# jjjkkyz/NU-NeRF

Hardware: AMD Instinct MI355X
Metric: train rays/sec (higher is better)
Workload: dtype f32

## Files before the change

### nu_nerf_amd/build.py

```python
import hashlib
import os
import subprocess
import sys

HERE = os.path.dirname(os.path.abspath(__file__))
CSRC = os.path.join(HERE, "csrc")
LIB = os.path.join(HERE, "libnunerf.so")
STAMP = os.path.join(HERE, ".libnunerf.stamp")
HIPCC = os.environ.get("HIPCC", "/opt/rocm/bin/hipcc")
FLAGS = ["--offload-arch=gfx950", "-O3", "-std=c++17", "-fPIC",
         "-fno-gpu-rdc", "-Wno-unused-result", "-I" + CSRC, "-I" + os.path.join(HERE, "..", "include")]
if os.environ.get("NU_BUILD_NO_PK_F32", "0") == "1":
    FLAGS += ["-Xclang", "-target-feature", "-Xclang", "-packed-fp32-ops"]


def _sources():
    return sorted(os.path.join(CSRC, f) for f in os.listdir(CSRC) if f.endswith(".hip"))


def _digest():
    h = hashlib.sha256()
    for f in sorted(os.listdir(CSRC)):
        if f.endswith((".hip", ".h")):
            with open(os.path.join(CSRC, f), "rb") as fh:
                h.update(f.encode())
                h.update(fh.read())
    inc = os.path.join(HERE, "..", "include", "nu_nerf.h")
    if os.path.exists(inc):
        with open(inc, "rb") as fh:
            h.update(fh.read())
    h.update(" ".join(FLAGS).encode())
    return h.hexdigest()


def build(force=False, verbose=True):
    dig = _digest()
    if not force and os.path.exists(LIB) and os.path.exists(STAMP):
        with open(STAMP) as fh:
            if fh.read().strip() == dig:
                return LIB
    objs = []
    procs = []
    objdir = os.path.join(HERE, "build")
    os.makedirs(objdir, exist_ok=True)
    for src in _sources():
        obj = os.path.join(objdir, os.path.basename(src)[:-4] + ".o")
        objs.append(obj)
        cmd = [HIPCC] + FLAGS + ["-c", src, "-o", obj]
        if verbose:
            print(" ".join(cmd), flush=True)
        procs.append((src, subprocess.Popen(cmd)))
    for src, p in procs:
        if p.wait() != 0:
            raise RuntimeError(f"hipcc failed on {src}")
    cmd = [HIPCC, "--offload-arch=gfx950", "-shared", "-fPIC", "-o", LIB] + objs
    if verbose:
        print(" ".join(cmd), flush=True)
    subprocess.check_call(cmd)
    with open(STAMP, "w") as fh:
        fh.write(dig)
    return LIB


if __name__ == "__main__":
    build(force="--force" in sys.argv)
    print(LIB)
```

### nu_nerf_amd/csrc/gemm_tn.hip

```cpp
#include "gemm_epi.h"

__device__ unsigned long long nu_dbg_clk[2];

#define NU_TN_BATCH_MAX 16
struct NuGemmTNBatch {
    NuGemmTN p[NU_TN_BATCH_MAX];
    int blk0[NU_TN_BATCH_MAX + 1];
    int n, pad_;
};
static __device__ __forceinline__ int tn_batch_decode(const NuGemmTNBatch& b, int tile_edge, int& bx, int& split) {
    int pi = 0;
    for (int i = 1; i < b.n; ++i) pi = ((int)blockIdx.x >= b.blk0[i]) ? i : pi;
    const int tiles = ((b.p[pi].N1 + tile_edge - 1) / tile_edge) * ((b.p[pi].N2 + tile_edge - 1) / tile_edge);
    const int local = (int)blockIdx.x - b.blk0[pi];
    split = local / tiles;
    bx = local - split * tiles;
    return pi;
}

template <bool BIG, int PREC>
static __device__ __forceinline__ void tn_body(const NuGemmTN& g, const int bx, const int split, const int grp) {
    constexpr bool BF16 = PREC == 1;
    constexpr bool SPLIT = PREC == 2;
    constexpr int kPlane = 128 * NT_LDSH;
    __shared__ __attribute__((aligned(16))) float smem[SPLIT ? 1 : 2][SPLIT ? 3 * kPlane : 128 * NT_LDS];
    __bf16* const hA = reinterpret_cast<__bf16*>(&smem[0][0]);
    __bf16* const hB = hA + (SPLIT ? 3 : 1) * kPlane;

    const int tid = threadIdx.x;
    const int lane = tid & 63;
    const int wid = tid >> 6;
    const int wr = wid >> 1, wc = wid & 1;
    const int t2 = (g.N2 + 127) / 128;
    const int n1t = bx / t2, n2t = bx - n1t * t2;
    const int n1_0 = n1t * 128, n2_0 = n2t * 128;
    const int N1p = ((g.N1 + 127) / 128) * 128, N2p = t2 * 128;

    int rows_per = (g.P + g.S - 1) / g.S;
    rows_per = ((rows_per + TBK - 1) / TBK) * TBK;
    const int p_begin = split * rows_per;
    int p_end = p_begin + rows_per;
    p_end = p_end < g.P ? p_end : g.P;
    const int ntile = p_end > p_begin ? (p_end - p_begin + TBK - 1) / TBK : 0;
    const int npair = g.A1 ? 2 : 1;
    const int total = ntile * npair;

    const int c = tid & 127;
    const int kg = tid >> 7;
    const bool do_bias = (g.bias_slab != nullptr) && (n2t == 0);

    f32x16 acc[2][2];
#pragma unroll
    for (int i = 0; i < 2; ++i)
#pragma unroll
        for (int j = 0; j < 2; ++j)
#pragma unroll
            for (int r = 0; r < 16; ++r) acc[i][j][r] = 0.0f;

    f32x4 ra4[4], rb4[4];
    int nvalid = 16;
    bool pend_pair0 = true;
    float bs = 0.f;
    auto load_tile = [&](int t) {
        const int pair = t >= ntile ? 1 : 0;
        const int kt = t - pair * ntile;
        const bool a16 = BF16 && (g.bf16 & (pair ? NU_TN_A1_16 : NU_TN_A0_16)) != 0;
        const bool b16 = BF16 && (g.bf16 & (pair ? NU_TN_B1_16 : NU_TN_B0_16)) != 0;
        const unsigned eA = a16 ? 2u : 4u, eB = b16 ? 2u : 4u;
        const char* __restrict__ A = (const char*)(pair ? g.A1 : g.A0) + (long long)grp * (pair ? g.sA1 : g.sA0) * eA;
        const char* __restrict__ B = (const char*)(pair ? g.B1 : g.B0) + (long long)grp * (pair ? g.sB1 : g.sB0) * eB;
        const int lda = pair ? g.lda1 : g.lda0;
        const int ldb = pair ? g.ldb1 : g.ldb0;
        int ca = n1_0 + c, cb = n2_0 + c;
        ca = ca < lda ? ca : lda - 1;
        cb = cb < ldb ? cb : ldb - 1;
        const int pbase = p_begin + kt * TBK + kg * 16;
        nvalid = p_end - pbase;
        pend_pair0 = pair == 0;
#pragma unroll
        for (int i = 0; i < 4; ++i)
#pragma unroll
            for (int e = 0; e < 4; ++e) {
                int pr = pbase + 4 * i + e;
                pr = pr < p_end ? pr : p_end - 1;
                const char* pa;
                const char* pb;
                if (BIG) {
                    pa = A + ((long long)pr * lda + ca) * eA;
                    pb = B + ((long long)pr * ldb + cb) * eB;
                } else {
                    pa = A + ((unsigned)pr * (unsigned)lda + (unsigned)ca) * eA;
                    pb = B + ((unsigned)pr * (unsigned)ldb + (unsigned)cb) * eB;
                }
                ra4[i][e] = a16 ? __uint_as_float((unsigned)*reinterpret_cast<const unsigned short*>(pa) << 16) : *reinterpret_cast<const float*>(pa);
                rb4[i][e] = b16 ? __uint_as_float((unsigned)*reinterpret_cast<const unsigned short*>(pb) << 16) : *reinterpret_cast<const float*>(pb);
            }
    };
    auto store_tile = [&]() {
#pragma unroll
        for (int i = 0; i < 4; ++i)
#pragma unroll
            for (int e = 0; e < 4; ++e) {
                const bool ok = 4 * i + e < nvalid;
                ra4[i][e] = ok ? ra4[i][e] : 0.f;
                rb4[i][e] = ok ? rb4[i][e] : 0.f;
            }
        if (do_bias && pend_pair0) {
#pragma unroll
            for (int i = 0; i < 4; ++i) bs += (ra4[i][0] + ra4[i][1]) + (ra4[i][2] + ra4[i][3]);
        }
#pragma unroll
        for (int i = 0; i < 4; ++i) {
            if (SPLIT) {
                bf16x4 p1, p2, p3;
                nu_split3(ra4[i], p1, p2, p3);
                __bf16* q = &hA[c * NT_LDSH + kg * 16 + 4 * i];
                *reinterpret_cast<bf16x4*>(q) = p1;
                *reinterpret_cast<bf16x4*>(q + kPlane) = p2;
                *reinterpret_cast<bf16x4*>(q + 2 * kPlane) = p3;
                nu_split3(rb4[i], p1, p2, p3);
                q = &hB[c * NT_LDSH + kg * 16 + 4 * i];
                *reinterpret_cast<bf16x4*>(q) = p1;
                *reinterpret_cast<bf16x4*>(q + kPlane) = p2;
                *reinterpret_cast<bf16x4*>(q + 2 * kPlane) = p3;
            } else if (BF16) {
                *reinterpret_cast<bf16x4*>(&hA[c * NT_LDSH + kg * 16 + 4 * i]) = nu_to_bf16x4(ra4[i]);
                *reinterpret_cast<bf16x4*>(&hB[c * NT_LDSH + kg * 16 + 4 * i]) = nu_to_bf16x4(rb4[i]);
            } else {
                float* s0 = &smem[0][0];
                *reinterpret_cast<f32x4*>(&s0[c * NT_LDS + kg * 16 + 4 * i]) = ra4[i];
                *reinterpret_cast<f32x4*>(&s0[128 * NT_LDS + c * NT_LDS + kg * 16 + 4 * i]) = rb4[i];
            }
        }
    };

    if (total > 0) {
        load_tile(0);
        store_tile();
    }
    __syncthreads();

    const int li = lane & 31, lh = lane >> 5;
    const int a_off = (wr * 64 + li) * NT_LDS + 4 * lh;
    const int b_off = (wc * 64 + li) * NT_LDS + 4 * lh;
    const int ah_off = (wr * 64 + li) * NT_LDSH + 8 * lh;
    const int bh_off = (wc * 64 + li) * NT_LDSH + 8 * lh;
    const int wr_u = __builtin_amdgcn_readfirstlane(wr), wc_u = __builtin_amdgcn_readfirstlane(wc);
    const bool vr0 = n1_0 + wr_u * 64 < g.N1, vr1 = n1_0 + wr_u * 64 + 32 < g.N1;
    const bool vc0 = n2_0 + wc_u * 64 < g.N2, vc1 = n2_0 + wc_u * 64 + 32 < g.N2;
    const bool v00 = vr0 && vc0, v01 = vr0 && vc1, v10 = vr1 && vc0, v11 = vr1 && vc1;
    for (int t = 0; t < total; ++t) {
        if (t + 1 < total) load_tile(t + 1);
        if (SPLIT) {
#pragma unroll
            for (int ks = 0; ks < 2; ++ks) {
// ... 501 lines not shown
            const bool ok = 4 * i + e < nvalid;
            ra4[i][e] = ok ? ra4[i][e] : 0.f;
            rb4[i][e] = ok ? rb4[i][e] : 0.f;
        }
        if (do_bias && pend_pair0) bs += (ra4[i][0] + ra4[i][1]) + (ra4[i][2] + ra4[i][3]);
        *reinterpret_cast<f32x4*>(&smem[st][0][c * NT_LDS + kg * 16 + 4 * i]) = ra4[i];
        *reinterpret_cast<f32x4*>(&smem[st][1][c * NT_LDS + kg * 16 + 4 * i]) = rb4[i];
    };
    auto load_tile = [&](int t) {
        load_begin(t);
#pragma unroll
        for (int i = 0; i < 4; ++i) load_piece(i, 0, 4);
        nvalid = nvalid_ld; pend_pair0 = pair0_ld;
    };
    auto store_tile = [&](int st) {
#pragma unroll
        for (int i = 0; i < 4; ++i) store_piece(st, i);
    };

    if (total > 0) {
        load_tile(0);
        store_tile(0);
        if (total > 1) load_tile(1);
    }
    __syncthreads();

    const int li = lane & 31, lh = lane >> 5;
    const int a_off = (wr * 64 + li) * NT_LDS + 4 * lh;
    const int b_off = (wc * 128 + li) * NT_LDS + 4 * lh;
    struct FragT { f32x4 a[2]; f32x4 b[4]; };
    FragT F0, F1;
    const int kg_u = __builtin_amdgcn_readfirstlane(kg);
    const char* rpA = nullptr;
    const char* rpB = nullptr;
    int prA = 0, prB = 0;
    auto ld_rows_begin = [&]() {
        int pr = ld_pbase_u + kg_u * 16;
        pr = pr < p_end ? pr : p_end - 1;
        prA = prB = pr;
        rpA = ldA + (long long)pr * ld_lda * 4;
        rpB = ldB + (long long)pr * ld_ldb * 4;
    };
    auto ld_one = [&](bool isA, int i, int e) {
        if (isA) {
            ra4[i][e] = *reinterpret_cast<const float*>(rpA + (unsigned)ld_ca * 4u);
            const bool more = prA + 1 < p_end;
            rpA += more ? (long long)ld_lda * 4 : 0;
            prA += more ? 1 : 0;
        } else {
            rb4[i][e] = *reinterpret_cast<const float*>(rpB + (unsigned)ld_cb * 4u);
            const bool more = prB + 1 < p_end;
            rpB += more ? (long long)ld_ldb * 4 : 0;
            prB += more ? 1 : 0;
        }
    };
    auto st_zero = [&](bool isA, int i) {
#pragma unroll
        for (int e = 0; e < 4; ++e) {
            if (isA) ra4[i][e] = (4 * i + e < nvalid) ? ra4[i][e] : 0.f;
            else rb4[i][e] = (4 * i + e < nvalid) ? rb4[i][e] : 0.f;
        }
    };
    bool bias_on = false;
    auto st_write = [&](bool isA, int st, int i) {
        if (isA) {
            const float rs = (ra4[i][0] + ra4[i][1]) + (ra4[i][2] + ra4[i][3]);
            bs += bias_on ? rs : 0.f;
            *reinterpret_cast<f32x4*>(&smem[st][0][c * NT_LDS + kg * 16 + 4 * i]) = ra4[i];
        } else {
            *reinterpret_cast<f32x4*>(&smem[st][1][c * NT_LDS + kg * 16 + 4 * i]) = rb4[i];
        }
    };
    int cur = 0;
    if (total > 0) {
#pragma unroll
        for (int i = 0; i < 2; ++i) F0.a[i] = *reinterpret_cast<const f32x4*>(&smem[0][0][a_off + 32 * i * NT_LDS]);
#pragma unroll
        for (int j = 0; j < 4; ++j) F0.b[j] = *reinterpret_cast<const f32x4*>(&smem[0][1][b_off + 32 * j * NT_LDS]);
    }
#define TN_PIN __builtin_amdgcn_sched_barrier(0);
#define TN_M(F, e, i, j) acc[i][j] = __builtin_amdgcn_mfma_f32_32x32x2f32(F.a[i][e], F.b[j][e], acc[i][j], 0, 0, 0); TN_PIN
#define TN_SLOT(F, e, ...) TN_SLOT_(F, e, __VA_ARGS__)
#define TN_SLOT_(F, e, X0, X1, X2, X3, X4, X5, X6)                                                   \
    TN_M(F, e, 0, 0) X0; TN_PIN TN_M(F, e, 0, 1) X1; TN_PIN TN_M(F, e, 0, 2) X2; TN_PIN TN_M(F, e, 0, 3) X3; TN_PIN     \
    TN_M(F, e, 1, 0) X4; TN_PIN TN_M(F, e, 1, 1) X5; TN_PIN TN_M(F, e, 1, 2) X6; TN_PIN TN_M(F, e, 1, 3)
#define TN_RDA(F, ST, kk, i) F.a[i] = *reinterpret_cast<const f32x4*>(&smem[ST][0][a_off + 32 * (i) * NT_LDS + (kk) * 8])
#define TN_RDB(F, ST, kk, j) F.b[j] = *reinterpret_cast<const f32x4*>(&smem[ST][1][b_off + 32 * (j) * NT_LDS + (kk) * 8])
#define TN_READS(F, ST, kk) TN_RDA(F, ST, kk, 0), TN_RDA(F, ST, kk, 1), TN_RDB(F, ST, kk, 0), TN_RDB(F, ST, kk, 1), TN_RDB(F, ST, kk, 2), TN_RDB(F, ST, kk, 3), (void)0
#define TN_LD2(i, e) ld_one(true, i, e), ld_one(false, i, e), ld_one(true, i, (e) + 1), ld_one(false, i, (e) + 1), (void)0, (void)0, (void)0
#define TN_ST(i) st_zero(true, i), st_write(true, cur ^ 1, i), st_zero(false, i), st_write(false, cur ^ 1, i), (void)0, (void)0, (void)0
    for (int t = 0; t < total; ++t) {
        bias_on = do_bias && pend_pair0 && t + 1 < total;
        load_begin(t + 2 < total ? t + 2 : total - 1);
        ld_rows_begin();
        TN_SLOT(F0, 0, TN_ST(0))
        TN_SLOT(F0, 1, TN_LD2(0, 0))
        TN_SLOT(F0, 2, TN_LD2(0, 2))
        TN_SLOT(F0, 3, TN_READS(F1, cur, 1))
        TN_SLOT(F1, 0, TN_ST(1))
        TN_SLOT(F1, 1, TN_LD2(1, 0))
        TN_SLOT(F1, 2, TN_LD2(1, 2))
        TN_SLOT(F1, 3, TN_READS(F0, cur, 2))
        TN_SLOT(F0, 0, TN_ST(2))
        TN_SLOT(F0, 1, TN_ST(3))
        TN_SLOT(F0, 2, TN_LD2(2, 0))
        TN_SLOT(F0, 3, TN_READS(F1, cur, 3))
        __syncthreads();
        TN_SLOT(F1, 0, TN_LD2(2, 2))
        TN_SLOT(F1, 1, TN_LD2(3, 0))
        TN_SLOT(F1, 2, TN_LD2(3, 2))
        TN_SLOT(F1, 3, TN_READS(F0, cur ^ 1, 0))
        nvalid = nvalid_ld; pend_pair0 = pair0_ld;
        cur ^= 1;
    }
#undef TN_PIN
#undef TN_M
#undef TN_SLOT
#undef TN_SLOT_
#undef TN_RDA
#undef TN_RDB
#undef TN_READS
#undef TN_LD2
#undef TN_ST

    float* __restrict__ slab = g.slab + (long long)grp * g.sSlab + (long long)split * N1p * N2p;
#pragma unroll
    for (int tm = 0; tm < 2; ++tm)
#pragma unroll
        for (int tn = 0; tn < 4; ++tn) {
            const int col = n2_0 + wc * 128 + tn * 32 + li;
#pragma unroll
            for (int r = 0; r < 16; ++r) {
                const int row = n1_0 + wr * 64 + tm * 32 + (r & 3) + 8 * (r >> 2) + 4 * lh;
                slab[(long long)row * N2p + col] = acc[tm][tn][r];
            }
        }
    if (do_bias) {
        float* red = &smem[0][0][0];
        red[kg * T + c] = bs;
        __syncthreads();
        if (tid < T) g.bias_slab[(long long)grp * g.sBiasSlab + (long long)split * N1p + n1_0 + tid] = red[tid] + red[T + tid];
    }
}

template <bool BIG>
__global__ __launch_bounds__(512, 2) void gemm_tn2_kernel(NuGemmTN g) { tn2_body<BIG>(g, blockIdx.x, blockIdx.y, blockIdx.z); }
template <bool BIG>
__global__ __launch_bounds__(512, 2) void gemm_tn2b_kernel(NuGemmTNBatch b) {
    int bx, split;
    const int pi = tn_batch_decode(b, 256, bx, split);
    tn2_body<BIG>(b.p[pi], bx, split, 0);
}

static bool nu_tn_big_tile(int N1, int N2, int groups, int prec, int S) {
    if ((prec & 3) == 2 || (N1 % 256) != 0 || (N2 % 256) != 0) return false;
    return (long long)(N1 / 256) * (N2 / 256) * (groups > 0 ? groups : 1) * S >= 192;
}
extern "C" int nu_wgrad_pick_split(int P, int N1, int N2, int groups, int prec) {
    if (groups < 1) groups = 1;
    const int rows_min = P <= 8192 ? 128 : 256;
    const int cap = (P + rows_min - 1) / rows_min > 0 ? (P + rows_min - 1) / rows_min : 1;
    if ((N1 % 256) == 0 && (N2 % 256) == 0) {
        int S = 256 / ((N1 / 256) * (N2 / 256) * groups);
        if (S < 1) S = 1;
        if (S > cap) S = cap;
        if (nu_tn_big_tile(N1, N2, groups, prec, S)) return S;
    }
    int S = 512 / (nu_cdiv(N1, 128) * nu_cdiv(N2, 128) * groups);
    if (S < 1) S = 1;
    if (S > cap) S = cap;
    return S;
}

int nu_gemm_tn_launch(const NuGemmTN& g, hipStream_t stream) {
    if (g.N1 <= 0 || g.N2 <= 0 || g.S <= 0) return NU_ERR_ARG;
    if ((g.lda0 & 3) || (g.ldb0 & 3) || (g.A1 && ((g.lda1 & 3) || (g.ldb1 & 3)))) return NU_ERR_ARG;
    const int prec = g.bf16 & 3;
    if (prec == 3 || ((g.bf16 & ~3) && prec != 1)) return NU_ERR_ARG;
    const bool big_tile = nu_tn_big_tile(g.N1, g.N2, g.groups, g.bf16, g.S);
    const long long max_ld = (g.lda0 > g.ldb0 ? g.lda0 : g.ldb0) > (g.A1 ? (g.lda1 > g.ldb1 ? g.lda1 : g.ldb1) : 0)
                                 ? (g.lda0 > g.ldb0 ? g.lda0 : g.ldb0) : (g.lda1 > g.ldb1 ? g.lda1 : g.ldb1);
    const bool big = (long long)g.P * max_ld * 4 >= (1LL << 32);
    if (prec == 0 && big_tile) {
        dim3 grid2((g.N1 / 256) * (g.N2 / 256), g.S, g.groups > 0 ? g.groups : 1);
        if (big) hipLaunchKernelGGL((gemm_tn2_kernel<true>), grid2, dim3(512), 0, stream, g);
        else hipLaunchKernelGGL((gemm_tn2_kernel<false>), grid2, dim3(512), 0, stream, g);
        return nu_launch_status();
    }
    dim3 grid(nu_cdiv(g.N1, 128) * nu_cdiv(g.N2, 128), g.S, g.groups > 0 ? g.groups : 1), block(256);
    if (prec == 1) {
        auto ok = [](const float* p, int ld, bool h) { return p == nullptr || ((((uintptr_t)p) & 15) == 0 && ld >= 8 && (!h || (ld & 7) == 0)); };
        const bool vec = ok(g.A0, g.lda0, g.bf16 & NU_TN_A0_16) && ok(g.B0, g.ldb0, g.bf16 & NU_TN_B0_16) &&
                         ok(g.A1, g.lda1, g.bf16 & NU_TN_A1_16) && ok(g.B1, g.ldb1, g.bf16 & NU_TN_B1_16) &&
                         ((g.sA0 | g.sB0 | g.sA1 | g.sB1) & 7) == 0;
        if (vec) {
            if (big_tile) {
                dim3 grid2((g.N1 / 256) * (g.N2 / 256), g.S, g.groups > 0 ? g.groups : 1);
                hipLaunchKernelGGL(gemm_tn16x256_kernel, grid2, dim3(512), 0, stream, g);
            } else {
                hipLaunchKernelGGL(gemm_tn16_kernel, grid, block, 0, stream, g);
            }
            return nu_launch_status();
        }
    }
    if (big) {
        if (prec == 2) hipLaunchKernelGGL((gemm_tn_kernel<true, 2>), grid, block, 0, stream, g);
        else if (prec == 1) hipLaunchKernelGGL((gemm_tn_kernel<true, 1>), grid, block, 0, stream, g);
        else hipLaunchKernelGGL((gemm_tn_kernel<true, 0>), grid, block, 0, stream, g);
    } else {
        if (prec == 2) hipLaunchKernelGGL((gemm_tn_kernel<false, 2>), grid, block, 0, stream, g);
        else if (prec == 1) hipLaunchKernelGGL((gemm_tn_kernel<false, 1>), grid, block, 0, stream, g);
        else hipLaunchKernelGGL((gemm_tn_kernel<false, 0>), grid, block, 0, stream, g);
    }
    return nu_launch_status();
}

struct NuReduceBatch {
    NuReduceDesc d[NU_REDUCE_MAX];
    int n;
};

__global__ __launch_bounds__(256) void slab_reduce_batched_kernel(NuReduceBatch b) {
    __shared__ float red[256];
    int di = 0;
    for (int i = 1; i < b.n; ++i) di = ((int)blockIdx.x >= b.d[i].blk_begin) ? i : di;
    const float* __restrict__ slab = b.d[di].slab;
    float* __restrict__ out = b.d[di].out;
    const int S = b.d[di].S, N1 = b.d[di].N1, N2 = b.d[di].N2, rs = b.d[di].rs, G = b.d[di].G;
    const long long ss = b.d[di].ss;
    const int opb = 256 / G;
    const int o = threadIdx.x % opb, g = threadIdx.x / opb;
    const int idx = ((int)blockIdx.x - b.d[di].blk_begin) * opb + o;
    const bool live = idx < N1 * N2;
    float v = 0.f;
    int n1 = 0, n2 = 0;
    if (live) {
        n1 = idx / N2;
        n2 = idx - n1 * N2;
        const float* p = slab + (long long)n1 * rs + n2;
        float s0 = 0.f, s1 = 0.f, s2 = 0.f, s3 = 0.f;
        int s = g;
        for (; s + 3 * G < S; s += 4 * G) {
            s0 += p[(long long)s * ss];
            s1 += p[(long long)(s + G) * ss];
            s2 += p[(long long)(s + 2 * G) * ss];
            s3 += p[(long long)(s + 3 * G) * ss];
        }
        for (; s < S; s += G) s0 += p[(long long)s * ss];
        v = (s0 + s1) + (s2 + s3);
    }
    if (G > 1) {
        red[threadIdx.x] = v;
        __syncthreads();
        if (g == 0)
            for (int gg = 1; gg < G; ++gg) v += red[gg * opb + o];
    }
    if (live && g == 0) {
        float* q = out + (long long)n1 * b.d[di].ldo + n2;
        v *= b.d[di].alpha;
        *q = b.d[di].accumulate ? *q + v : v;
    }
}

static int nu_reduce_launch_chunk(const NuReduceDesc* descs, int n, hipStream_t stream) {
    NuReduceBatch b;
    int blocks = 0;
    for (int i = 0; i < n; ++i) {
        b.d[i] = descs[i];
        const long long nout = (long long)descs[i].N1 * descs[i].N2;
        int G = 1;
        while (G < 16 && nout * G < 16384 && 2 * G <= descs[i].S) G *= 2;
        b.d[i].G = G;
        b.d[i].blk_begin = blocks;
        blocks += (int)nu_cdivl(nout, 256 / G);
    }
    b.n = n;
    if (blocks <= 0) return NU_OK;
    hipLaunchKernelGGL(slab_reduce_batched_kernel, dim3(blocks), dim3(256), 0, stream, b);
    return nu_launch_status();
}

extern "C" int nu_slab_reduce_batched(const NuReduceDesc* descs, int n, hipStream_t stream) {
    int i = 0;
    while (i < n) {
        if (descs[i].N1 <= 0 || descs[i].N2 <= 0 || descs[i].S <= 0) return NU_ERR_ARG;
        int j = i + 1;
        if (!descs[i].accumulate)
            while (j < n && j - i < NU_REDUCE_MAX && !descs[j].accumulate) ++j;
        const int rc = nu_reduce_launch_chunk(descs + i, j - i, stream);
        if (rc) return rc;
        i = j;
    }
    return NU_OK;
}

int nu_reduce_push(NuReduceDesc* descs, int* ndesc, int cap, const float* slab, int S, int N1, int N2, int rs,
                   long long ss, float* out, int ldo, float alpha, int accumulate) {
    if (*ndesc >= cap) return NU_ERR_WORKSPACE;
    NuReduceDesc& d = descs[(*ndesc)++];
    d.slab = slab; d.out = out; d.ss = ss; d.S = S; d.N1 = N1; d.N2 = N2; d.rs = rs; d.ldo = ldo;
    d.accumulate = accumulate; d.G = 1; d.blk_begin = 0; d.alpha = alpha;
    return NU_OK;
}

extern "C" int nu_gemm_nt(const float* A, int lda, const float* B, int ldb, int M, int N, int K, float* C, int ldc,
                          float* C2, int ldc2, const float* bias, const float* H, int ldh, const float* D, int ldd,
                          const float* Cadd, int ldadd, int zero_to, float alpha, int epi, hipStream_t stream) {
    NuGemmNT g = {};
    g.A = A; g.lda = lda; g.B = B; g.ldb = ldb; g.M = M; g.N = N; g.K = K;
    g.C = C; g.ldc = ldc; g.C2 = C2; g.ldc2 = ldc2; g.bias = bias; g.H = H; g.ldh = ldh; g.D = D; g.ldd = ldd;
    g.Cadd = Cadd; g.ldadd = ldadd; g.zero_to = zero_to; g.alpha = alpha; g.groups = 1; g.epi = epi;
    return nu_gemm_nt_launch(g, stream);
}

extern "C" long long nu_gemm_tn_workspace_bytes(int N1, int N2, int S) {
    return (long long)S * nu_rup(N1, 128) * (nu_rup(N2, 128) + 1) * sizeof(float);
}

extern "C" int nu_gemm_tn(const float* A0, int lda0, const float* B0, int ldb0, const float* A1, int lda1,
                          const float* B1, int ldb1, int P, int N1, int N2, float* C, int ldc, float* bias_out,
                          int S, void* workspace, long long workspace_bytes, hipStream_t stream) {
    NuGemmTN g = {};
    g.A0 = A0; g.lda0 = lda0; g.B0 = B0; g.ldb0 = ldb0; g.A1 = A1; g.lda1 = lda1; g.B1 = B1; g.ldb1 = ldb1;
    g.P = P; g.N1 = N1; g.N2 = N2; g.S = S; g.groups = 1;
    return nu_wgrad(&g, C, ldc, 0, bias_out, 0, workspace, workspace_bytes, stream);
}

extern "C" int nu_gemm_nt_size(void) { return (int)sizeof(NuGemmNT); }
extern "C" int nu_gemm_tn_size(void) { return (int)sizeof(NuGemmTN); }

extern "C" int nu_gemm_nt_ex(const NuGemmNT* g, hipStream_t stream) { return nu_gemm_nt_launch(*g, stream); }

extern "C" long long nu_wgrad_workspace_bytes(int N1, int N2, int S, int groups) {
    return (long long)(groups > 0 ? groups : 1) * S * nu_rup(N1, 128) * (nu_rup(N2, 128) + 1) * sizeof(float);
}
extern "C" int nu_wgrad_enqueue(const NuGemmTN* gin, float* dW, int ldw, long long sW, float* db, long long sDb,
                                void* workspace, long long workspace_bytes, NuReduceDesc* descs, int* ndesc, int cap,
                                hipStream_t stream) {
    NuGemmTN g = *gin;
    const int groups = g.groups > 0 ? g.groups : 1;
    if (g.P <= 0) return NU_ERR_ARG;
    if (workspace_bytes < nu_wgrad_workspace_bytes(g.N1, g.N2, g.S, groups)) return NU_ERR_WORKSPACE;
    if (*ndesc + groups * (db ? 2 : 1) > cap) return NU_ERR_WORKSPACE;
    const int N1p = nu_rup(g.N1, 128), N2p = nu_rup(g.N2, 128);
    const long long slab_per = (long long)g.S * N1p * N2p;
    const long long bias_per = (long long)g.S * N1p;
    g.slab = (float*)workspace;
    g.sSlab = slab_per;
    g.bias_slab = db ? g.slab + slab_per * groups : nullptr;
    g.sBiasSlab = bias_per;
    g.groups = groups;
    int rc = nu_gemm_tn_launch(g, stream);
    for (int z = 0; z < groups && rc == NU_OK; ++z) {
        rc = nu_reduce_push(descs, ndesc, cap, g.slab + z * slab_per, g.S, g.N1, g.N2, N2p, (long long)N1p * N2p,
                            dW + z * sW, ldw, 1.0f, 0);
        if (rc == NU_OK && db)
            rc = nu_reduce_push(descs, ndesc, cap, g.bias_slab + z * bias_per, g.S, g.N1, 1, 1, N1p, db + z * sDb, 1, 1.0f, 0);
    }
    return rc;
}

extern "C" int nu_wgrad(const NuGemmTN* gin, float* dW, int ldw, long long sW, float* db, long long sDb,
                        void* workspace, long long workspace_bytes, hipStream_t stream) {
    const int groups = gin->groups > 0 ? gin->groups : 1;
    if (groups > NU_REDUCE_MAX / 2) return NU_ERR_ARG;
    NuReduceDesc descs[NU_REDUCE_MAX];
    int n = 0;
    int rc = nu_wgrad_enqueue(gin, dW, ldw, sW, db, sDb, workspace, workspace_bytes, descs, &n, NU_REDUCE_MAX, stream);
    if (rc) return rc;
    return nu_slab_reduce_batched(descs, n, stream);
}

extern "C" int nu_wgrad_item_size(void) { return (int)sizeof(NuWgradItem); }

static int ctx_reduce_now(NuOpCtx* c, hipStream_t stream) {
    if (c->ndesc > 0) {
        const int rc = nu_slab_reduce_batched(c->descs, c->ndesc, stream);
        if (rc != NU_OK) return rc;
        c->ndesc = 0;
    }
    c->arena_off = 0;
    return NU_OK;
}
extern "C" int nu_wgrad_flush(NuOpCtx* c, hipStream_t stream);
extern "C" int nu_ctx_reduce(NuOpCtx* c, hipStream_t stream) { return ctx_reduce_now(c, stream); }
extern "C" int nu_ctx_flush(NuOpCtx* c, hipStream_t stream) {
    const int rc = nu_wgrad_flush(c, stream);
    if (rc != NU_OK) return rc;
    return ctx_reduce_now(c, stream);
}
int nu_ctx_take(NuOpCtx* c, long long nbytes, int ndesc_needed, hipStream_t stream, float** out, long long* out_bytes) {
    const long long n = (nbytes + 255) / 256 * 64;
    if (n > c->arena_floats) return NU_ERR_WORKSPACE;
    if (c->arena_off + n > c->arena_floats || c->ndesc + ndesc_needed > c->cap) {
        if (c->forked) return NU_ERR_WORKSPACE;
        const int rc = ctx_reduce_now(c, stream);
        if (rc != NU_OK) return rc;
    }
    *out = c->arena + c->arena_off;
    *out_bytes = n * 4;
    c->arena_off += n;
    return NU_OK;
}
void nu_ctx_ev_begin(NuOpCtx* c, hipStream_t stream) {
    if (c->ev && c->nev + 2 <= c->ev_cap) (void)hipEventRecord(static_cast<hipEvent_t>(c->ev[c->nev]), stream);
}
void nu_ctx_ev_end(NuOpCtx* c, hipStream_t stream, double kind, double flops, double bytes) {
    if (c->ev && c->nev + 2 <= c->ev_cap) {
        (void)hipEventRecord(static_cast<hipEvent_t>(c->ev[c->nev + 1]), stream);
        double* m = c->ev_meta + 3 * (c->nev / 2);
        m[0] = kind; m[1] = flops; m[2] = bytes;
        c->nev += 2;
    }
}

static inline bool tn_item_big(const NuGemmTN& g) {
    const long long m0 = g.lda0 > g.ldb0 ? g.lda0 : g.ldb0, m1 = g.A1 ? (g.lda1 > g.ldb1 ? g.lda1 : g.ldb1) : 0;
    return (long long)g.P * (m0 > m1 ? m0 : m1) * 4 >= (1LL << 32);
}

static int wgrad_launch_batch(NuOpCtx* c, NuWgradItem* it, const int* idx, int m, int klass, hipStream_t stream) {
    long long bytes = 0;
    int ndesc = 0, nprob = 0;
    for (int k = 0; k < m; ++k) {
        const NuGemmTN& g = it[idx[k]].g;
        bytes += (nu_wgrad_workspace_bytes(g.N1, g.N2, g.S, g.groups) + 255) / 256 * 256;
        ndesc += g.groups * (it[idx[k]].db ? 2 : 1);
        nprob += g.groups;
    }
    if (nprob > NU_TN_BATCH_MAX) return NU_ERR_ARG;
    float* ws;
    long long nb;
    int rc = nu_ctx_take(c, bytes, ndesc, stream, &ws, &nb);
    if (rc != NU_OK) return rc;
    NuGemmTNBatch b;
    int np = 0, blocks = 0;
    double flops = 0, abytes = 0;
    const int edge = klass == 2 ? 256 : 128;
    for (int k = 0; k < m; ++k) {
        NuWgradItem& w = it[idx[k]];
        const NuGemmTN& g = w.g;
        const int N1p = nu_rup(g.N1, 128), N2p = nu_rup(g.N2, 128);
        const long long slab_per = (long long)g.S * N1p * N2p, bias_per = (long long)g.S * N1p;
        float* slab = ws;
        float* bias_slab = w.db ? slab + slab_per * g.groups : nullptr;
        ws += (nu_wgrad_workspace_bytes(g.N1, g.N2, g.S, g.groups) + 255) / 256 * 64;
        for (int z = 0; z < g.groups; ++z) {
            NuGemmTN& q = b.p[np];
            q = g;
            q.groups = 1;
            q.A0 = g.A0 + z * g.sA0; q.B0 = g.B0 + z * g.sB0;
            q.A1 = g.A1 ? g.A1 + z * g.sA1 : nullptr; q.B1 = g.B1 ? g.B1 + z * g.sB1 : nullptr;
            q.slab = slab + z * slab_per; q.bias_slab = bias_slab ? bias_slab + z * bias_per : nullptr;
            q.sSlab = 0; q.sBiasSlab = 0;
            b.blk0[np++] = blocks;
            blocks += nu_cdiv(g.N1, edge) * nu_cdiv(g.N2, edge) * g.S;
            rc = nu_reduce_push(c->descs, &c->ndesc, c->cap, q.slab, g.S, g.N1, g.N2, N2p, (long long)N1p * N2p, w.dW + z * w.sW, w.ldw, 1.0f, 0);
            if (rc == NU_OK && w.db)
                rc = nu_reduce_push(c->descs, &c->ndesc, c->cap, q.bias_slab, g.S, g.N1, 1, 1, N1p, w.db + z * w.sDb, 1, 1.0f, 0);
            if (rc != NU_OK) return rc;
        }
        flops += w.flops; abytes += w.bytes;
    }
    b.blk0[np] = blocks;
    b.n = np; b.pad_ = 0;
    nu_ctx_ev_begin(c, stream);
    if (klass == 2) hipLaunchKernelGGL((gemm_tn2b_kernel<false>), dim3(blocks), dim3(512), 0, stream, b);
    else hipLaunchKernelGGL((gemm_tnb_kernel<false>), dim3(blocks), dim3(256), 0, stream, b);
    rc = nu_launch_status();
    nu_ctx_ev_end(c, stream, 1.0, flops, abytes);
    return rc;
}

static int wgrad_launch_single(NuOpCtx* c, NuWgradItem& w, hipStream_t stream) {
    NuGemmTN& g = w.g;
    g.S = nu_wgrad_pick_split(g.P, g.N1, g.N2, g.groups, g.bf16 & 3);
    float* ws;
    long long nb;
    int rc = nu_ctx_take(c, nu_wgrad_workspace_bytes(g.N1, g.N2, g.S, g.groups), 2 * g.groups, stream, &ws, &nb);
    if (rc != NU_OK) return rc;
    nu_ctx_ev_begin(c, stream);
    rc = nu_wgrad_enqueue(&g, w.dW, w.ldw, w.sW, w.db, w.sDb, ws, nb, c->descs, &c->ndesc, c->cap, stream);
    nu_ctx_ev_end(c, stream, 1.0, w.flops, w.bytes);
    return rc;
}

extern "C" int nu_wgrad_flush(NuOpCtx* c, hipStream_t stream) {
    const int n = c->npend;
    if (n <= 0 || c->pend == nullptr) return NU_OK;
    NuWgradItem* it = c->pend;
    c->npend = 0;
    int klass[NU_WGRAD_QUEUE_MAX];
    if (n > NU_WGRAD_QUEUE_MAX) return NU_ERR_ARG;
    int pmax = 0;
    for (int i = 0; i < n; ++i) {
        NuGemmTN& g = it[i].g;
        if (g.groups < 1) g.groups = 1;
        klass[i] = ((g.bf16 & 3) == 0 && (g.bf16 & ~3) == 0 && !tn_item_big(g) && g.groups <= NU_TN_BATCH_MAX) ? 1 : 0;
        if (klass[i] && g.P > pmax) pmax = g.P;
    }
    const int rows_min = pmax <= 8192 ? 128 : 256;
    auto plan = [&](int k, int edge, int target) -> long long {
        long long work = 0;
        for (int i = 0; i < n; ++i)
            if (klass[i] == k) work += (long long)it[i].g.P * nu_cdiv(it[i].g.N1, edge) * nu_cdiv(it[i].g.N2, edge) * it[i].g.groups;
        if (work == 0) return 0;
        long long rows = nu_cdivl(work, target);
        rows = rows < rows_min ? rows_min : rows;
        rows = nu_cdivl(rows, TBK) * TBK;
        while (true) {
            long long wgs = 0;
            for (int i = 0; i < n; ++i)
                if (klass[i] == k) wgs += nu_cdivl(it[i].g.P, rows) * nu_cdiv(it[i].g.N1, edge) * nu_cdiv(it[i].g.N2, edge) * it[i].g.groups;
            if (wgs <= target || rows >= (1LL << 30)) { for (int i = 0; i < n; ++i) if (klass[i] == k) it[i].g.S = (int)nu_cdivl(it[i].g.P, rows); return wgs; }
            rows += TBK;
        }
    };
    for (int i = 0; i < n; ++i)
        if (klass[i] == 1 && (it[i].g.N1 % 256) == 0 && (it[i].g.N2 % 256) == 0) klass[i] = 2;
    if (plan(2, 256, 256) < 192)
        for (int i = 0; i < n; ++i) if (klass[i] == 2) klass[i] = 1;
    plan(1, 128, 1024);
    for (int i = 0; i < n; ++i)
        if (klass[i] == 0) { const int rc = wgrad_launch_single(c, it[i], stream); if (rc != NU_OK) return rc; }
    for (int k = 2; k >= 1; --k) {
        int idx[NU_WGRAD_QUEUE_MAX], m = 0, nprob = 0;
        long long bytes = 0;
        for (int i = 0; i <= n; ++i) {
            const bool mine = i < n && klass[i] == k;
            long long need = 0;
            if (mine) need = (nu_wgrad_workspace_bytes(it[i].g.N1, it[i].g.N2, it[i].g.S, it[i].g.groups) + 255) / 256 * 256;
            const bool full = mine && m > 0 && (nprob + it[i].g.groups > NU_TN_BATCH_MAX || bytes + need > c->arena_floats * 4);
            if ((i == n || full) && m > 0) {
                const int rc = wgrad_launch_batch(c, it, idx, m, k, stream);
                if (rc != NU_OK) return rc;
                m = 0; nprob = 0; bytes = 0;
            }
            if (mine) { idx[m++] = i; nprob += it[i].g.groups; bytes += need; }
        }
    }
    return NU_OK;
}

extern "C" int nu_wgrad_defer(NuOpCtx* c, const NuGemmTN* g, float* dW, int ldw, long long sW, float* db, long long sDb, double flops,
                              double bytes, hipStream_t stream) {
    if (g->P <= 0) return NU_OK;
    NuWgradItem w;
    w.g = *g; w.dW = dW; w.ldw = ldw; w.pad_ = 0; w.sW = sW; w.db = db; w.sDb = sDb; w.flops = flops; w.bytes = bytes;
    if (w.g.groups < 1) w.g.groups = 1;
    if (c->pend == nullptr || c->pend_cap <= 0) return wgrad_launch_single(c, w, stream);
    if (c->npend >= c->pend_cap || c->npend >= NU_WGRAD_QUEUE_MAX) {
        const int rc = nu_wgrad_flush(c, stream);
        if (rc != NU_OK) return rc;
    }
    c->pend[c->npend++] = w;
    return NU_OK;
}

__global__ __launch_bounds__(256) void mfma_peak_kernel(float* out, int iters) {
    f32x16 a0 = {}, a1 = {}, a2 = {}, a3 = {};
    const unsigned long long c0 = clock64(), w0 = wall_clock64();
    float x = (float)threadIdx.x * 1e-3f, y = 1.0f + (float)blockIdx.x * 1e-6f;
    for (int i = 0; i < iters; ++i) {
        a0 = __builtin_amdgcn_mfma_f32_32x32x2f32(x, y, a0, 0, 0, 0);
        a1 = __builtin_amdgcn_mfma_f32_32x32x2f32(y, x, a1, 0, 0, 0);
        a2 = __builtin_amdgcn_mfma_f32_32x32x2f32(x, x, a2, 0, 0, 0);
        a3 = __builtin_amdgcn_mfma_f32_32x32x2f32(y, y, a3, 0, 0, 0);
    }
    float s = 0.f;
    for (int r = 0; r < 16; ++r) s += a0[r] + a1[r] + a2[r] + a3[r];
    if (s == 123.456f) out[0] = s;
    if (blockIdx.x == 0 && threadIdx.x == 0) { nu_dbg_clk[0] = clock64() - c0; nu_dbg_clk[1] = wall_clock64() - w0; }
}
extern "C" double nu_debug_clock_mhz(void) {
    unsigned long long h[2] = {0, 0};
    if (hipMemcpyFromSymbol(h, HIP_SYMBOL(nu_dbg_clk), sizeof(h)) != hipSuccess || h[1] == 0) return -1.0;
    return (double)h[0] / (double)h[1] * 100.0;
}
extern "C" int nu_debug_mfma_peak(float* out, int blocks, int iters, hipStream_t stream) {
    hipLaunchKernelGGL(mfma_peak_kernel, dim3(blocks), dim3(256), 0, stream, out, iters);
    return nu_launch_status();
}
```

Before: 99220.

## Add software-pipelined vec4 fp32 wgrad TN kernel for aligned 256-tile batches

Adds a new tn3 weight-gradient kernel for 256x256 tiles. It uses vectorized f32x4 global loads, double-buffered padded LDS and a hand-scheduled MFMA loop that interleaves fragment reads, bias partial sums and global prefetch two tiles ahead. Batches that qualify for the big-tile class and have 16-byte-aligned operands are routed to it, aiming to hide load latency behind MFMA issue. The clock-probe debug symbol is also moved behind a build flag. The manual scheduling with sched_barrier and the row clamping for tail tiles add correctness risk and register pressure.

```diff
diff --git a/nu_nerf_amd/build.py b/nu_nerf_amd/build.py
--- a/nu_nerf_amd/build.py
+++ b/nu_nerf_amd/build.py
@@ -12,6 +12,8 @@
          "-fno-gpu-rdc", "-Wno-unused-result", "-I" + CSRC, "-I" + os.path.join(HERE, "..", "include")]
 if os.environ.get("NU_BUILD_NO_PK_F32", "0") == "1":
     FLAGS += ["-Xclang", "-target-feature", "-Xclang", "-packed-fp32-ops"]
+if os.environ.get("NU_BUILD_CLOCK_PROBE", "0") == "1":
+    FLAGS += ["-DNU_CLOCK_PROBE"]
 
 
 def _sources():
diff --git a/nu_nerf_amd/csrc/gemm_tn.hip b/nu_nerf_amd/csrc/gemm_tn.hip
--- a/nu_nerf_amd/csrc/gemm_tn.hip
+++ b/nu_nerf_amd/csrc/gemm_tn.hip
@@ -1,6 +1,8 @@
 #include "gemm_epi.h"
 
+#ifdef NU_CLOCK_PROBE
 __device__ unsigned long long nu_dbg_clk[2];
+#endif
 
 #define NU_TN_BATCH_MAX 16
 struct NuGemmTNBatch {
@@ -808,6 +810,192 @@
     tn2_body<BIG>(b.p[pi], bx, split, 0);
 }
 
+#define TN3_RS 264
+static __device__ __forceinline__ void tn3_body(const NuGemmTN& g, const int bx, const int split, const int grp) {
+    constexpr int T = 256;
+    __shared__ __attribute__((aligned(16))) float smem[2][2][TBK * TN3_RS];
+    const int tid = threadIdx.x;
+    const int lane = tid & 63;
+    const int wid = __builtin_amdgcn_readfirstlane(tid >> 6);
+    const int wr = wid >> 1, wc = wid & 1;
+    const int t2 = g.N2 / T;
+    const int n1t = bx / t2, n2t = bx - n1t * t2;
+    const int n1_0 = n1t * T, n2_0 = n2t * T;
+    const int N1p = g.N1, N2p = g.N2;
+
+    int rows_per = (g.P + g.S - 1) / g.S;
+    rows_per = ((rows_per + TBK - 1) / TBK) * TBK;
+    const int p_begin = split * rows_per;
+    int p_end = p_begin + rows_per;
+    p_end = p_end < g.P ? p_end : g.P;
+    const int ntile = p_end > p_begin ? (p_end - p_begin + TBK - 1) / TBK : 0;
+    const int npair = g.A1 ? 2 : 1;
+    const int total = ntile * npair;
+
+    const int c = tid & (T - 1);
+    const int kg = tid / T;
+    const bool do_bias = (g.bias_slab != nullptr) && (n2t == 0);
+
+    f32x16 acc[2][4];
+#pragma unroll
+    for (int i = 0; i < 2; ++i)
+#pragma unroll
+        for (int j = 0; j < 4; ++j)
+#pragma unroll
+            for (int r = 0; r < 16; ++r) acc[i][j][r] = 0.0f;
+
+    f32x4 ra4[4], rb4[4];
+    int nvalid = TBK, nvalid_ld = TBK;
+    const char* rpA = nullptr;
+    const char* rpB = nullptr;
+    long long strA = 0, strB = 0;
+    int prA = 0, prB = 0;
+    auto load_begin = [&](int t) {
+        const int pair = t >= ntile ? 1 : 0;
+        const int kt = t - pair * ntile;
+        const char* A = (const char*)(pair ? g.A1 + (long long)grp * g.sA1 : g.A0 + (long long)grp * g.sA0);
+        const char* B = (const char*)(pair ? g.B1 + (long long)grp * g.sB1 : g.B0 + (long long)grp * g.sB0);
+        strA = (long long)(pair ? g.lda1 : g.lda0) * 4;
+        strB = (long long)(pair ? g.ldb1 : g.ldb0) * 4;
+        const int pbase = p_begin + kt * TBK;
+        nvalid_ld = p_end - pbase;
+        int pr = pbase + 4 * wid;
+        pr = pr < p_end ? pr : p_end - 1;
+        prA = prB = pr;
+        rpA = A + pr * strA + (long long)n1_0 * 4;
+        rpB = B + pr * strB + (long long)n2_0 * 4;
+    };
+    auto ld_one = [&](bool isA, int i) {
+        if (isA) {
+            ra4[i] = *reinterpret_cast<const f32x4*>(rpA + (unsigned)lane * 16u);
+            const bool more = prA + 1 < p_end;
+            rpA += more ? strA : 0;
+            prA += more ? 1 : 0;
+        } else {
+            rb4[i] = *reinterpret_cast<const f32x4*>(rpB + (unsigned)lane * 16u);
+            const bool more = prB + 1 < p_end;
+            rpB += more ? strB : 0;
+            prB += more ? 1 : 0;
+        }
+    };
+    auto st_one = [&](bool isA, int st, int i) {
+        const bool ok = 4 * wid + i < nvalid;
+        f32x4 v = isA ? ra4[i] : rb4[i];
+#pragma unroll
+        for (int e = 0; e < 4; ++e) v[e] = ok ? v[e] : 0.f;
+        *reinterpret_cast<f32x4*>(&smem[st][isA ? 0 : 1][(4 * wid + i) * TN3_RS + 4 * lane]) = v;
+    };
+
+    if (total > 0) {
+        load_begin(0);
+#pragma unroll
+        for (int i = 0; i < 4; ++i) { ld_one(true, i); ld_one(false, i); }
+        nvalid = nvalid_ld;
+#pragma unroll
+        for (int i = 0; i < 4; ++i) { st_one(true, 0, i); st_one(false, 0, i); }
+        if (total > 1) {
+            load_begin(1);
+#pragma unroll
+            for (int i = 0; i < 4; ++i) { ld_one(true, i); ld_one(false, i); }
+            nvalid = nvalid_ld;
+        }
+    }
+    __syncthreads();
+
+    const int li = lane & 31, lh = lane >> 5;
+    const int a_off = 4 * lh * TN3_RS + wr * 64 + li;
+    const int b_off = 4 * lh * TN3_RS + wc * 128 + li;
+    const int s_off = 16 * kg * TN3_RS + c;
+    struct Frag3 { float a[2]; float b[4]; };
+    Frag3 F0, F1;
+    float bs = 0.f, bq[4] = {0.f, 0.f, 0.f, 0.f};
+    bool bias_on = false;
+    int cur = 0;
+    constexpr int kOp = TBK * TN3_RS, kStage = 2 * kOp;
+    const float* const S = &smem[0][0][0];
+    if (total > 0) {
+#pragma unroll
+        for (int i = 0; i < 2; ++i) F0.a[i] = S[a_off + 32 * i];
+#pragma unroll
+        for (int j = 0; j < 4; ++j) F0.b[j] = S[kOp + b_off + 32 * j];
+    }
+#define TN3_PIN __builtin_amdgcn_sched_barrier(0);
+#define TN3_M(F, i, j) acc[i][j] = __builtin_amdgcn_mfma_f32_32x32x2f32(F.a[i], F.b[j], acc[i][j], 0, 0, 0); TN3_PIN
+#define TN3_ROW(s) ((8 * ((s) >> 2) + ((s) & 3)) * TN3_RS)
+#define TN3_SLOT(F, G, AP, BP, sn, X0, X1, X6)                                                              \
+    TN3_M(F, 0, 0) G.a[0] = S[AP + TN3_ROW(sn)]; X0; TN3_PIN                                             \
+    TN3_M(F, 0, 1) G.b[0] = S[BP + TN3_ROW(sn)]; X1; TN3_PIN                                             \
+    TN3_M(F, 0, 2) G.b[1] = S[BP + TN3_ROW(sn) + 32]; TN3_PIN                                            \
+    TN3_M(F, 0, 3) G.b[2] = S[BP + TN3_ROW(sn) + 64]; TN3_PIN                                            \
+    TN3_M(F, 1, 0) G.b[3] = S[BP + TN3_ROW(sn) + 96]; TN3_PIN                                            \
+    TN3_M(F, 1, 1) G.a[1] = S[AP + TN3_ROW(sn) + 32]; TN3_PIN                                            \
+    TN3_M(F, 1, 2) X6; TN3_PIN                                                                               \
+    TN3_M(F, 1, 3)
+#define TN3_BQ(q, r) bq[q] = S[sc + (r) * TN3_RS]
+#define TN3_BSUM { const float rs = (bq[0] + bq[1]) + (bq[2] + bq[3]); bs += bias_on ? rs : 0.f; }
+    for (int t = 0; t < total; ++t) {
+        bias_on = do_bias && t < ntile;
+        load_begin(t + 2 < total ? t + 2 : total - 1);
+        const int Ac = cur * kStage + a_off, Bc = cur * kStage + kOp + b_off;
+        const int An = (cur ^ 1) * kStage + a_off, Bn = (cur ^ 1) * kStage + kOp + b_off;
+        const int sc = cur * kStage + s_off;
+        TN3_SLOT(F0, F1, Ac, Bc, 1, TN3_BQ(0, 0), TN3_BQ(1, 1), st_one(true, cur ^ 1, 0))
+        TN3_SLOT(F1, F0, Ac, Bc, 2, TN3_BQ(2, 2), TN3_BQ(3, 3), st_one(false, cur ^ 1, 0))
+        TN3_BSUM
+        TN3_SLOT(F0, F1, Ac, Bc, 3, TN3_BQ(0, 4), TN3_BQ(1, 5), ld_one(true, 0))
+        TN3_SLOT(F1, F0, Ac, Bc, 4, TN3_BQ(2, 6), TN3_BQ(3, 7), ld_one(false, 0))
+        TN3_BSUM
+        TN3_SLOT(F0, F1, Ac, Bc, 5, TN3_BQ(0, 8), TN3_BQ(1, 9), st_one(true, cur ^ 1, 1))
+        TN3_SLOT(F1, F0, Ac, Bc, 6, TN3_BQ(2, 10), TN3_BQ(3, 11), st_one(false, cur ^ 1, 1))
+        TN3_BSUM
+        TN3_SLOT(F0, F1, Ac, Bc, 7, TN3_BQ(0, 12), TN3_BQ(1, 13), ld_one(true, 1))
+        TN3_SLOT(F1, F0, Ac, Bc, 8, TN3_BQ(2, 14), TN3_BQ(3, 15), ld_one(false, 1))
+        TN3_BSUM
+        TN3_SLOT(F0, F1, Ac, Bc, 9, (void)0, (void)0, st_one(true, cur ^ 1, 2))
+        TN3_SLOT(F1, F0, Ac, Bc, 10, (void)0, (void)0, st_one(false, cur ^ 1, 2))
+        TN3_SLOT(F0, F1, Ac, Bc, 11, (void)0, (void)0, ld_one(true, 2))
+        TN3_SLOT(F1, F0, Ac, Bc, 12, (void)0, (void)0, ld_one(false, 2))
+        TN3_SLOT(F0, F1, Ac, Bc, 13, (void)0, (void)0, st_one(true, cur ^ 1, 3))
+        TN3_SLOT(F1, F0, Ac, Bc, 14, (void)0, (void)0, st_one(false, cur ^ 1, 3))
+        TN3_SLOT(F0, F1, Ac, Bc, 15, (void)0, (void)0, ld_one(true, 3))
+        __syncthreads();
+        TN3_SLOT(F1, F0, An, Bn, 0, (void)0, (void)0, ld_one(false, 3))
+        nvalid = nvalid_ld;
+        cur ^= 1;
+    }
+#undef TN3_PIN
+#undef TN3_M
+#undef TN3_ROW
+#undef TN3_SLOT
+#undef TN3_BQ
+#undef TN3_BSUM
+
+    float* __restrict__ slab = g.slab + (long long)grp * g.sSlab + (long long)split * N1p * N2p;
+#pragma unroll
+    for (int tm = 0; tm < 2; ++tm)
+#pragma unroll
+        for (int tn = 0; tn < 4; ++tn) {
+            const int col = n2_0 + wc * 128 + tn * 32 + li;
+#pragma unroll
+            for (int r = 0; r < 16; ++r) {
+                const int row = n1_0 + wr * 64 + tm * 32 + (r & 3) + 8 * (r >> 2) + 4 * lh;
+                slab[(long long)row * N2p + col] = acc[tm][tn][r];
+            }
+        }
+    if (do_bias) {
+        float* red = &smem[0][0][0];
+        red[kg * T + c] = bs;
+        __syncthreads();
+        if (tid < T) g.bias_slab[(long long)grp * g.sBiasSlab + (long long)split * N1p + n1_0 + tid] = red[tid] + red[T + tid];
+    }
+}
+
+__global__ __launch_bounds__(512, 2) void gemm_tn3b_kernel(NuGemmTNBatch b) {
+    int bx, split;
+    const int pi = tn_batch_decode(b, 256, bx, split);
+    tn3_body(b.p[pi], bx, split, 0);
+}
+
 static bool nu_tn_big_tile(int N1, int N2, int groups, int prec, int S) {
     if ((prec & 3) == 2 || (N1 % 256) != 0 || (N2 % 256) != 0) return false;
     return (long long)(N1 / 256) * (N2 / 256) * (groups > 0 ? groups : 1) * S >= 192;
@@ -1075,6 +1263,11 @@
     return (long long)g.P * (m0 > m1 ? m0 : m1) * 4 >= (1LL << 32);
 }
 
+static inline bool tn_item_vec4(const NuGemmTN& g) {
+    auto ok = [](const float* p, int ld, long long s) { return p == nullptr || ((((uintptr_t)p) & 15) == 0 && (ld & 3) == 0 && (s & 3) == 0); };
+    return ok(g.A0, g.lda0, g.sA0) && ok(g.B0, g.ldb0, g.sB0) && ok(g.A1, g.lda1, g.sA1) && ok(g.B1, g.ldb1, g.sB1);
+}
+
 static int wgrad_launch_batch(NuOpCtx* c, NuWgradItem* it, const int* idx, int m, int klass, hipStream_t stream) {
     long long bytes = 0;
     int ndesc = 0, nprob = 0;
@@ -1092,7 +1285,7 @@
     NuGemmTNBatch b;
     int np = 0, blocks = 0;
     double flops = 0, abytes = 0;
-    const int edge = klass == 2 ? 256 : 128;
+    const int edge = klass >= 2 ? 256 : 128;
     for (int k = 0; k < m; ++k) {
         NuWgradItem& w = it[idx[k]];
         const NuGemmTN& g = w.g;
@@ -1121,7 +1314,8 @@
     b.blk0[np] = blocks;
     b.n = np; b.pad_ = 0;
     nu_ctx_ev_begin(c, stream);
-    if (klass == 2) hipLaunchKernelGGL((gemm_tn2b_kernel<false>), dim3(blocks), dim3(512), 0, stream, b);
+    if (klass == 3) hipLaunchKernelGGL(gemm_tn3b_kernel, dim3(blocks), dim3(512), 0, stream, b);
+    else if (klass == 2) hipLaunchKernelGGL((gemm_tn2b_kernel<false>), dim3(blocks), dim3(512), 0, stream, b);
     else hipLaunchKernelGGL((gemm_tnb_kernel<false>), dim3(blocks), dim3(256), 0, stream, b);
     rc = nu_launch_status();
     nu_ctx_ev_end(c, stream, 1.0, flops, abytes);
@@ -1178,8 +1372,10 @@
         for (int i = 0; i < n; ++i) if (klass[i] == 2) klass[i] = 1;
     plan(1, 128, 1024);
     for (int i = 0; i < n; ++i)
+        if (klass[i] == 2 && tn_item_vec4(it[i].g)) klass[i] = 3;
+    for (int i = 0; i < n; ++i)
         if (klass[i] == 0) { const int rc = wgrad_launch_single(c, it[i], stream); if (rc != NU_OK) return rc; }
-    for (int k = 2; k >= 1; --k) {
+    for (int k = 3; k >= 1; --k) {
         int idx[NU_WGRAD_QUEUE_MAX], m = 0, nprob = 0;
         long long bytes = 0;
         for (int i = 0; i <= n; ++i) {
@@ -1226,12 +1422,20 @@
     float s = 0.f;
     for (int r = 0; r < 16; ++r) s += a0[r] + a1[r] + a2[r] + a3[r];
     if (s == 123.456f) out[0] = s;
+#ifdef NU_CLOCK_PROBE
     if (blockIdx.x == 0 && threadIdx.x == 0) { nu_dbg_clk[0] = clock64() - c0; nu_dbg_clk[1] = wall_clock64() - w0; }
+#else
+    (void)c0; (void)w0;
+#endif
 }
 extern "C" double nu_debug_clock_mhz(void) {
+#ifdef NU_CLOCK_PROBE
     unsigned long long h[2] = {0, 0};
     if (hipMemcpyFromSymbol(h, HIP_SYMBOL(nu_dbg_clk), sizeof(h)) != hipSuccess || h[1] == 0) return -1.0;
     return (double)h[0] / (double)h[1] * 100.0;
+#else
+    return -1.0;
+#endif
 }
 extern "C" int nu_debug_mfma_peak(float* out, int blocks, int iters, hipStream_t stream) {
     hipLaunchKernelGGL(mfma_peak_kernel, dim3(blocks), dim3(256), 0, stream, out, iters);
```

New measurement: 99640 (median of 6 runs). About the same (+0.4%).
